# espiriki/Garbage_Classification_RCA

Hardware: AMD Instinct MI355X
Metric: train samples/sec (image+text pairs), MM-RCA ViT-B16+DistilBERT (higher is better)
Workload: dtype bf16

## Files before the change

garbage_classification_rca_amd/csrc/attention_cls.hip:

```cpp
#include "common.h"

#define CLS_MAX_S 1024
#define CLS_MAX_DH 128

template <typename T>
__device__ __forceinline__ float dot_lds(const T* __restrict__ row, const float* __restrict__ vec, int dh) {
  float a = 0.f;
  for (int d = 0; d < dh; d += 4) {
    Vec4<T> v = Vec4<T>::load(row + d);
    a += v.v[0] * vec[d] + v.v[1] * vec[d + 1] + v.v[2] * vec[d + 2] + v.v[3] * vec[d + 3];
  }
  return a;
}

__device__ __forceinline__ float block_reduce(float x, float* red, bool is_max) {
  const int wave = threadIdx.x >> 6, lane = threadIdx.x & 63;
  x = is_max ? wave_max(x) : wave_sum(x);
  __syncthreads();
  if (lane == 0) red[wave] = x;
  __syncthreads();
  return is_max ? fmaxf(fmaxf(red[0], red[1]), fmaxf(red[2], red[3])) : (red[0] + red[1] + red[2] + red[3]);
}

template <typename T>
__global__ void __launch_bounds__(256)
mha_cls_fwd_k(const T* __restrict__ qkv, const int32_t* __restrict__ key_mask, T* __restrict__ out, float* __restrict__ lse,
              int B, int H, int Smax, int dh, float scale, float drop_p, uint64_t drop_seed, const int32_t* __restrict__ cu) {
  __shared__ float qv[CLS_MAX_DH], p[CLS_MAX_S], red[4], part[4][CLS_MAX_DH];
  const float drop_sc = drop_p > 0.f ? 1.f / (1.f - drop_p) : 1.f;
  const int b = blockIdx.x / H, h = blockIdx.x % H, tid = threadIdx.x;
  const int row0 = cu ? cu[b] : b * Smax, S = cu ? cu[b + 1] - cu[b] : Smax;
  if (S <= 0) return;
  const int64_t ld = 3LL * H * dh;
  const T* Q = qkv + (int64_t)row0 * ld + h * dh;
  const T* Kp = Q + H * dh;
  const T* Vp = Kp + H * dh;
  for (int d = tid; d < dh; d += 256) qv[d] = to_f(Q[d]);
  __syncthreads();
  float m = -INFINITY;
  for (int j = tid; j < S; j += 256) {
    float s = -INFINITY;
    if (!key_mask || key_mask[row0 + j] != 0) s = dot_lds(Kp + (int64_t)j * ld, qv, dh) * scale;
    p[j] = s;
    m = fmaxf(m, s);
  }
  m = block_reduce(m, red, true);
  float l = 0.f;
  for (int j = tid; j < S; j += 256) {
    const float e = m > -INFINITY ? __expf(p[j] - m) : 0.f;
    l += e;
    p[j] = (drop_p > 0.f && mmrca_uniform(drop_seed, ((uint64_t)blockIdx.x * Smax + 0) * Smax + j) < drop_p) ? 0.f : e * drop_sc;
  }
  l = block_reduce(l, red, false);
  const float inv = l > 0.f ? 1.f / l : 0.f;
  const int ncg = dh / 4, slices = 256 / ncg;
  const int cg = tid % ncg, sl = tid / ncg;
  float o[4] = {0.f, 0.f, 0.f, 0.f};
  if (sl < slices) {
    for (int j = sl; j < S; j += slices) {
      const float pj = p[j];
      Vec4<T> v = Vec4<T>::load(Vp + (int64_t)j * ld + cg * 4);
#pragma unroll
      for (int r = 0; r < 4; ++r) o[r] += pj * v.v[r];
    }
  }
  for (int off = ncg; off < 64; off <<= 1) {
#pragma unroll
    for (int r = 0; r < 4; ++r) o[r] += __shfl_xor(o[r], off, 64);
  }
  const int wave = tid >> 6, lane = tid & 63;
  if (lane < ncg) {
#pragma unroll
    for (int r = 0; r < 4; ++r) part[wave][lane * 4 + r] = o[r];
  }
  __syncthreads();
  for (int d = tid; d < dh; d += 256)
    out[(int64_t)b * (H * dh) + h * dh + d] = from_f<T>((part[0][d] + part[1][d] + part[2][d] + part[3][d]) * inv);
  if (tid == 0) lse[blockIdx.x] = l > 0.f ? m + __logf(l) : INFINITY;
}

template <typename T>
__global__ void __launch_bounds__(256)
mha_cls_bwd_k(const T* __restrict__ qkv, const int32_t* __restrict__ key_mask, const T* __restrict__ out,
              const T* __restrict__ dout, const float* __restrict__ lse, T* __restrict__ dqkv,
              int B, int H, int Smax, int dh, float scale, float drop_p, uint64_t drop_seed, const int32_t* __restrict__ cu) {
  __shared__ float qv[CLS_MAX_DH], dov[CLS_MAX_DH], pk[CLS_MAX_S], ds[CLS_MAX_S], red[4], part[4][CLS_MAX_DH];
  const float drop_sc = drop_p > 0.f ? 1.f / (1.f - drop_p) : 1.f;
  const int b = blockIdx.x / H, h = blockIdx.x % H, tid = threadIdx.x;
  const int row0 = cu ? cu[b] : b * Smax, S = cu ? cu[b + 1] - cu[b] : Smax;
  if (S <= 0) return;
  const int64_t ld = 3LL * H * dh;
  const T* Q = qkv + (int64_t)row0 * ld + h * dh;
  const T* Kp = Q + H * dh;
  const T* Vp = Kp + H * dh;
  T* dQ = dqkv + (int64_t)row0 * ld + h * dh;
  T* dK = dQ + H * dh;
  T* dV = dK + H * dh;
  float dsum = 0.f;
  for (int d = tid; d < dh; d += 256) {
    qv[d] = to_f(Q[d]);
    const float g = to_f(dout[(int64_t)b * (H * dh) + h * dh + d]);
    dov[d] = g;
    dsum += g * to_f(out[(int64_t)b * (H * dh) + h * dh + d]);
  }
  dsum = block_reduce(dsum, red, false);
  const float Lse = lse[blockIdx.x];
  for (int j = tid; j < S; j += 256) {
    float pkj = 0.f, dsj = 0.f;
    if (!key_mask || key_mask[row0 + j] != 0) {
      const float s = dot_lds(Kp + (int64_t)j * ld, qv, dh) * scale;
      const float pj = __expf(s - Lse);
      const float dp = dot_lds(Vp + (int64_t)j * ld, dov, dh);
      const float keep = drop_p > 0.f ? (mmrca_uniform(drop_seed, ((uint64_t)blockIdx.x * Smax + 0) * Smax + j) >= drop_p ? drop_sc : 0.f) : 1.f;
      dsj = pj * (dp * keep - dsum) * scale;
      pkj = pj * keep;
    }
    pk[j] = pkj; ds[j] = dsj;
  }
  __syncthreads();
  const int ncg = dh / 4, slices = 256 / ncg;
  const int cg = tid % ncg, sl = tid / ncg;
  float qa[4] = {0.f, 0.f, 0.f, 0.f};
  if (sl < slices) {
    float dor[4], qr[4];
#pragma unroll
    for (int r = 0; r < 4; ++r) { dor[r] = dov[cg * 4 + r]; qr[r] = qv[cg * 4 + r]; }
    for (int j = sl; j < S; j += slices) {
      const float pkj = pk[j], dsj = ds[j];
      Vec4<T> k = Vec4<T>::load(Kp + (int64_t)j * ld + cg * 4), ov, ok, oz;
#pragma unroll
      for (int r = 0; r < 4; ++r) { ov.v[r] = pkj * dor[r]; ok.v[r] = dsj * qr[r]; oz.v[r] = 0.f; qa[r] += dsj * k.v[r]; }
      ov.store(dV + (int64_t)j * ld + cg * 4);
      ok.store(dK + (int64_t)j * ld + cg * 4);
      if (j > 0) oz.store(dQ + (int64_t)j * ld + cg * 4);
    }
  }
  for (int off = ncg; off < 64; off <<= 1) {
#pragma unroll
    for (int r = 0; r < 4; ++r) qa[r] += __shfl_xor(qa[r], off, 64);
  }
  const int wave = tid >> 6, lane = tid & 63;
  if (lane < ncg) {
#pragma unroll
    for (int r = 0; r < 4; ++r) part[wave][lane * 4 + r] = qa[r];
  }
  __syncthreads();
  for (int d = tid; d < dh; d += 256) dQ[d] = from_f<T>(part[0][d] + part[1][d] + part[2][d] + part[3][d]);
}

static bool cls_shape_ok(int S, int dh) {
  return S <= CLS_MAX_S && dh <= CLS_MAX_DH && (dh == 16 || dh == 32 || dh == 64 || dh == 128);
}

extern "C" int mmrca_mha_cls_fwd(const void* qkv, const int32_t* key_mask, void* out, float* lse, int B, int H, int S, int dh,
                                 float scale, float drop_p, uint64_t drop_seed, const int32_t* cu_seqlens, int dtype, void* stream) {
  MMRCA_REQUIRE(qkv && out && lse, "mha_cls_fwd: null pointer");
  MMRCA_REQUIRE(drop_p >= 0.f && drop_p < 1.f, "mha_cls_fwd: dropout p must be in [0,1)");
  MMRCA_REQUIRE(B > 0 && H > 0 && S > 0 && cls_shape_ok(S, dh), "mha_cls_fwd: B=%d H=%d S=%d dh=%d unsupported", B, H, S, dh);
  MMRCA_DISPATCH_DTYPE(dtype, "mha_cls_fwd",
    hipLaunchKernelGGL(mha_cls_fwd_k<T>, dim3(B * H), dim3(256), 0, (hipStream_t)stream, (const T*)qkv, key_mask, (T*)out, lse,
                       B, H, S, dh, scale, drop_p, drop_seed, cu_seqlens);)
  MMRCA_CHECK_LAUNCH("mha_cls_fwd");
  return 0;
}

extern "C" int mmrca_mha_cls_bwd(const void* qkv, const int32_t* key_mask, const void* out, const void* dout, const float* lse,
                                 void* dqkv, int B, int H, int S, int dh, float scale, float drop_p, uint64_t drop_seed,
                                 const int32_t* cu_seqlens, int dtype, void* stream) {
  MMRCA_REQUIRE(qkv && out && dout && lse && dqkv, "mha_cls_bwd: null pointer");
  MMRCA_REQUIRE(drop_p >= 0.f && drop_p < 1.f, "mha_cls_bwd: dropout p must be in [0,1)");
  MMRCA_REQUIRE(B > 0 && H > 0 && S > 0 && cls_shape_ok(S, dh), "mha_cls_bwd: B=%d H=%d S=%d dh=%d unsupported", B, H, S, dh);
  MMRCA_DISPATCH_DTYPE(dtype, "mha_cls_bwd",
    hipLaunchKernelGGL(mha_cls_bwd_k<T>, dim3(B * H), dim3(256), 0, (hipStream_t)stream, (const T*)qkv, key_mask, (const T*)out,
                       (const T*)dout, lse, (T*)dqkv, B, H, S, dh, scale, drop_p, drop_seed, cu_seqlens);)
  MMRCA_CHECK_LAUNCH("mha_cls_bwd");
  return 0;
}

MMRCA_SEED_EPOCH_EXPORT(attention_cls)
```

garbage_classification_rca_amd/csrc/gemm.hip:

```cpp
#include "common.h"
#include "lds_asm.h"

typedef __attribute__((ext_vector_type(4))) float f32x4;

template <typename T>
__global__ void __launch_bounds__(256)
gemm_ref_k(const T* __restrict__ A, const T* __restrict__ B, void* __restrict__ Cv, const T* __restrict__ bias,
           const T* __restrict__ addend, T* __restrict__ preact, int64_t M, int64_t N, int64_t K,
           int64_t sam, int64_t sak, int64_t sbn, int64_t sbk, int64_t ldc, int act, int accum) {
  __shared__ float As[16][65], Bs[16][65];
  const int tx = threadIdx.x & 15, ty = threadIdx.x >> 4;
  const int64_t m0 = (int64_t)blockIdx.y * 64, n0 = (int64_t)blockIdx.x * 64;
  float acc[4][4], mid[4][4];
#pragma unroll
  for (int i = 0; i < 4; ++i)
#pragma unroll
    for (int j = 0; j < 4; ++j) acc[i][j] = mid[i][j] = 0.f;
  int blk = 0;
  for (int64_t k0 = 0; k0 < K; k0 += 16) {
#pragma unroll
    for (int i = 0; i < 4; ++i) {
      const int idx = threadIdx.x + i * 256;
      int mm, kk;
      if (sak == 1) { mm = idx >> 4; kk = idx & 15; } else { kk = idx >> 6; mm = idx & 63; }
// ... 857 lines not shown
      if (seg == 2) Bp = B_lo;
    }
    if (!ATOMIC_F32 && !X3 && t == nt - 1 && ((kend - kbeg) & (GBK - 1)) != 0) {
      stage_tile<A_KROW, 1>(Ap, lda, m_blk, M, kbeg + (int64_t)t * GBK, smem, wave, lane, kend);
      stage_tile<B_KROW, 2>(Bp, ldb, n_blk, N, kbeg + (int64_t)t * GBK, smem + TILE_BYTES, wave, lane, kend);
    } else {
      stage_tile<A_KROW>(Ap, lda, m_blk, M, kbeg + (int64_t)t * GBK, smem, wave, lane);
      stage_tile<B_KROW>(Bp, ldb, n_blk, N, kbeg + (int64_t)t * GBK, smem + TILE_BYTES, wave, lane);
    }
    asm volatile("s_waitcnt vmcnt(0)" ::: "memory");
    __syncthreads();
#pragma unroll
    for (int ks = 0; ks < 2; ++ks) {
      bf16x8 af[4], bfr[4];
#pragma unroll
      for (int i = 0; i < 4; ++i) af[i] = load_frag<A_KROW>(smem, wr * 64 + i * 16, ks, lane);
#pragma unroll
      for (int j = 0; j < 4; ++j) bfr[j] = load_frag<B_KROW>(smem + TILE_BYTES, wc * 64 + j * 16, ks, lane);
#pragma unroll
      for (int i = 0; i < 4; ++i)
#pragma unroll
        for (int j = 0; j < 4; ++j) {
          if (ATOMIC_F32) acc[i][j] = __builtin_amdgcn_mfma_f32_16x16x32_bf16(af[i], bfr[j], acc[i][j], 0, 0, 0);
          else            acc[i][j] = __builtin_amdgcn_mfma_f32_16x16x32_bf16(bfr[j], af[i], acc[i][j], 0, 0, 0);
        }
    }
    __syncthreads();
  }
  const int g = lane >> 4, l16 = lane & 15;
  if (ATOMIC_F32) {
    float* C = (float*)Cv;
#pragma unroll
    for (int i = 0; i < 4; ++i)
#pragma unroll
      for (int j = 0; j < 4; ++j) {
        const int64_t n = n_blk + wc * 64 + j * 16 + l16;
#pragma unroll
        for (int r = 0; r < 4; ++r) {
          const int64_t m = m_blk + wr * 64 + i * 16 + 4 * g + r;
          if (m < M && n < N) atomicAdd(C + m * ldc + n, acc[i][j][r]);
        }
      }
  } else if constexpr (X3) {
    const float* biasf = reinterpret_cast<const float*>(bias);
    const float* addf = reinterpret_cast<const float*>(addend);
    float* pref = reinterpret_cast<float*>(preact);
    constexpr int EP_STRIDE = 128 * 4 + 16;
    const int half = lane >> 5, l32 = lane & 31;
    const int64_t ncol = n_blk + l32 * 4;
    f32x4 bv = (f32x4){0.f, 0.f, 0.f, 0.f};
    if (biasf) bv = *reinterpret_cast<const f32x4*>(biasf + ncol);
    const float* side = act == MMRCA_ACT_MUL ? pref : addf;
    float cs[4] = {0.f, 0.f, 0.f, 0.f};
#pragma unroll
    for (int i = 0; i < 4; ++i) {
      f32x4 sd[4];
      if (side) {
#pragma unroll
        for (int rr = 0; rr < 4; ++rr) {
          const int lrow = wave * 8 + rr * 2 + half;
          int64_t m = m_blk + (lrow >> 4) * 64 + i * 16 + (lrow & 15);
          if (m > M - 1) m = M - 1;
          sd[rr] = *reinterpret_cast<const f32x4*>(side + m * ldc + ncol);
        }
      }
#pragma unroll
      for (int j = 0; j < 4; ++j)
        *reinterpret_cast<f32x4*>(smem + (wr * 16 + l16) * EP_STRIDE + (wc * 64 + j * 16 + 4 * g) * 4) = acc[i][j];
      __syncthreads();
#pragma unroll
      for (int rr = 0; rr < 4; ++rr) {
        const int lrow = wave * 8 + rr * 2 + half;
        const int64_t m = m_blk + (lrow >> 4) * 64 + i * 16 + (lrow & 15);
        if (m < M && ncol < N) {
          const f32x4 c = *reinterpret_cast<const f32x4*>(smem + lrow * EP_STRIDE + l32 * 16);
          float v[4] = {c[0] + bv[0], c[1] + bv[1], c[2] + bv[2], c[3] + bv[3]};
          if (act == MMRCA_ACT_MUL) {
#pragma unroll
            for (int r = 0; r < 4; ++r) v[r] *= sd[rr][r];
          } else if (act == MMRCA_ACT_GELU_SAVE_GRAD) {
            float dg[4];
            gelu_and_grad_fast4(v, dg);
            if (pre16) {
              bf16x4 o16;
#pragma unroll
              for (int r = 0; r < 4; ++r) o16[r] = (bf16_t)dg[r];
              *reinterpret_cast<bf16x4*>(preact + m * ldc + ncol) = o16;
            } else {
              *reinterpret_cast<f32x4*>(pref + m * ldc + ncol) = (f32x4){dg[0], dg[1], dg[2], dg[3]};
            }
          } else if (act == MMRCA_ACT_GELU_BWD) {
            const f32x4 h4 = *reinterpret_cast<const f32x4*>(pref + m * ldc + ncol);
#pragma unroll
            for (int r = 0; r < 4; ++r) v[r] *= gelu_grad_f(h4[r]);
          } else if (pref) {
            *reinterpret_cast<f32x4*>(pref + m * ldc + ncol) = (f32x4){v[0], v[1], v[2], v[3]};
          }
          if (act == MMRCA_ACT_GELU) gelu_fast4(v);
          if (addf) {
            if (act == MMRCA_ACT_MUL) {
              const f32x4 a4 = *reinterpret_cast<const f32x4*>(addf + m * ldc + ncol);
#pragma unroll
              for (int r = 0; r < 4; ++r) v[r] += a4[r];
            } else {
#pragma unroll
              for (int r = 0; r < 4; ++r) v[r] += sd[rr][r];
            }
          }
          if (C_lo) {
            bf16x4 hi, lo;
#pragma unroll
            for (int r = 0; r < 4; ++r) { hi[r] = (bf16_t)v[r]; lo[r] = (bf16_t)(v[r] - (float)hi[r]); cs[r] += (float)hi[r] + (float)lo[r]; }
            *reinterpret_cast<bf16x4*>(reinterpret_cast<bf16_t*>(Cv) + m * ldc + ncol) = hi;
            *reinterpret_cast<bf16x4*>(C_lo + m * ldc + ncol) = lo;
          } else {
#pragma unroll
            for (int r = 0; r < 4; ++r) cs[r] += v[r];
            *reinterpret_cast<f32x4*>(reinterpret_cast<float*>(Cv) + m * ldc + ncol) = (f32x4){v[0], v[1], v[2], v[3]};
          }
        }
      }
      __syncthreads();
    }
    if (colsum) {
      float* red = reinterpret_cast<float*>(smem);
#pragma unroll
      for (int r = 0; r < 4; ++r) red[(wave * 2 + half) * 128 + l32 * 4 + r] = cs[r];
      __syncthreads();
      if (threadIdx.x < 128) {
        float t = 0.f;
#pragma unroll
        for (int q = 0; q < 8; ++q) t += red[q * 128 + threadIdx.x];
        if (n_blk + threadIdx.x < N) atomicAdd(colsum + n_blk + threadIdx.x, t);
      }
    }
  } else {
    bf16_t* C = (bf16_t*)Cv;
    constexpr int EP_STRIDE = 128 * 4 + 16;
    const int half = lane >> 5, l32 = lane & 31;
    const int64_t ncol = n_blk + l32 * 4;
    float bv[4] = {0.f, 0.f, 0.f, 0.f};
    if (bias) {
      bf16x4 b4 = *reinterpret_cast<const bf16x4*>(bias + (ncol < N ? ncol : N - 4));
#pragma unroll
      for (int r = 0; r < 4; ++r) bv[r] = (float)b4[r];
    }
    bf16x4 add4[4][4];
    const bf16_t* side = act == MMRCA_ACT_MUL ? preact : addend;
    if (side) {
#pragma unroll
      for (int i = 0; i < 4; ++i)
#pragma unroll
        for (int rr = 0; rr < 4; ++rr) {
          const int lrow = wave * 8 + rr * 2 + half;
          int64_t m = m_blk + (lrow >> 4) * 64 + i * 16 + (lrow & 15);
          if (m > M - 1) m = M - 1;
          add4[i][rr] = *reinterpret_cast<const bf16x4*>(side + m * ldc + ncol);
        }
    }
    float cs[4] = {0.f, 0.f, 0.f, 0.f};
    [[maybe_unused]] float st2[4] = {0.f, 0.f, 0.f, 0.f}, stsh[4] = {0.f, 0.f, 0.f, 0.f};
    if constexpr (BNS) {
      if (bst.shift && ncol < N) {
#pragma unroll
        for (int r = 0; r < 4; ++r) stsh[r] = bst.shift[ncol + r];
      }
    }
#pragma unroll
    for (int i = 0; i < 4; ++i) {
#pragma unroll
      for (int j = 0; j < 4; ++j)
        *reinterpret_cast<f32x4*>(smem + (wr * 16 + l16) * EP_STRIDE + (wc * 64 + j * 16 + 4 * g) * 4) = acc[i][j];
      __syncthreads();
#pragma unroll
      for (int rr = 0; rr < 4; ++rr) {
        const int lrow = wave * 8 + rr * 2 + half;
        const int64_t m = m_blk + (lrow >> 4) * 64 + i * 16 + (lrow & 15);
        if (m < M && ncol < N) {
          const f32x4 c = *reinterpret_cast<const f32x4*>(smem + lrow * EP_STRIDE + l32 * 16);
          float v[4] = {c[0] + bv[0], c[1] + bv[1], c[2] + bv[2], c[3] + bv[3]};
          if (act == MMRCA_ACT_MUL) {
#pragma unroll
            for (int r = 0; r < 4; ++r) v[r] *= (float)add4[i][rr][r];
          } else if (act == MMRCA_ACT_GELU_SAVE_GRAD) {
            bf16x4 o;
            float dg[4];
            gelu_and_grad_fast4(v, dg);
#pragma unroll
            for (int r = 0; r < 4; ++r) o[r] = (bf16_t)dg[r];
            *reinterpret_cast<bf16x4*>(preact + m * ldc + ncol) = o;
          } else if (act == MMRCA_ACT_GELU_BWD) {
            bf16x4 h4 = *reinterpret_cast<const bf16x4*>(preact + m * ldc + ncol);
#pragma unroll
            for (int r = 0; r < 4; ++r) v[r] *= gelu_grad_f((float)h4[r]);
          } else if (preact) {
            bf16x4 o;
#pragma unroll
            for (int r = 0; r < 4; ++r) o[r] = (bf16_t)v[r];
            *reinterpret_cast<bf16x4*>(preact + m * ldc + ncol) = o;
          }
          if (act == MMRCA_ACT_GELU) {
            gelu_fast4(v);
          }
          if (addend) {
            if (act == MMRCA_ACT_MUL) {
              bf16x4 a4 = *reinterpret_cast<const bf16x4*>(addend + m * ldc + ncol);
#pragma unroll
              for (int r = 0; r < 4; ++r) v[r] += (float)a4[r];
            } else {
#pragma unroll
              for (int r = 0; r < 4; ++r) v[r] += (float)add4[i][rr][r];
            }
          }
          bf16x4 o;
#pragma unroll
          for (int r = 0; r < 4; ++r) {
            o[r] = (bf16_t)v[r];
            if constexpr (BNS) { const float d = (float)o[r] - stsh[r]; cs[r] += d; st2[r] = fmaf(d, d, st2[r]); }
            else cs[r] += (float)o[r];
          }
          *reinterpret_cast<bf16x4*>(C + m * ldc + ncol) = o;
        }
      }
      __syncthreads();
    }
    if constexpr (BNS) {
      float* red = reinterpret_cast<float*>(smem);
#pragma unroll
      for (int r = 0; r < 4; ++r) { red[(wave * 2 + half) * 128 + l32 * 4 + r] = cs[r]; red[1024 + (wave * 2 + half) * 128 + l32 * 4 + r] = st2[r]; }
      __syncthreads();
      const int col = threadIdx.x & 127, which = threadIdx.x >> 7;
      float t = 0.f;
#pragma unroll
      for (int q = 0; q < 8; ++q) t += red[which * 1024 + q * 128 + col];
      if (n_blk + col < N) (which ? bst.s2 : bst.s1)[(int64_t)tm * N + n_blk + col] = t;
    } else if (colsum) {
      float* red = reinterpret_cast<float*>(smem);
#pragma unroll
      for (int r = 0; r < 4; ++r) red[(wave * 2 + half) * 128 + l32 * 4 + r] = cs[r];
      __syncthreads();
      if (threadIdx.x < 128) {
        float t = 0.f;
#pragma unroll
        for (int q = 0; q < 8; ++q) t += red[q * 128 + threadIdx.x];
        if (n_blk + threadIdx.x < N) atomicAdd(colsum + n_blk + threadIdx.x, t);
      }
    }
  }
}

template <bool AK, bool BK2, bool AT, int WPE, bool X3 = false, bool BNS = false, bool F4 = false>
static void launch_mfma1s(const void* A, const void* B, void* C, const void* bias, const void* addend, void* preact,
                          int64_t M, int64_t N, int64_t K, int64_t lda, int64_t ldb, int64_t ldc, int act, int tiles_m,
                          int tiles_n, int ksplits, int64_t ksplit_len, float* colsum, hipStream_t st,
                          const void* A_lo = nullptr, const void* B_lo = nullptr, void* C_lo = nullptr, int nseg = 3,
                          BnStat bst = BnStat{nullptr, nullptr, nullptr}, int pre16 = 0) {
  hipLaunchKernelGGL((gemm_mfma_k1s<AK, BK2, AT, WPE, X3, BNS, F4>), dim3(tiles_m * tiles_n, ksplits), dim3(256), 2 * TILE_BYTES, st,
                     (const bf16_t*)A, (const bf16_t*)B, C, (const bf16_t*)bias, (const bf16_t*)addend, (bf16_t*)preact,
                     M, N, K, lda, ldb, ldc, act, tiles_m, tiles_n, ksplit_len, colsum, (const bf16_t*)A_lo, (const bf16_t*)B_lo,
                     (bf16_t*)C_lo, nseg, bst, pre16);
}

static void wgrad_ksplit(int64_t K, int64_t tiles, int64_t target, int& ksplits, int64_t& ksplit_len) {
  const int64_t ksteps = K / GBK;
  int64_t want = target / tiles;
  if (want < 1) want = 1;
  if (want > ksteps / 4) want = ksteps / 4 > 0 ? ksteps / 4 : 1;
  const int64_t steps_per = (ksteps + want - 1) / want;
  ksplit_len = steps_per * GBK;
  ksplits = (int)((ksteps + steps_per - 1) / steps_per);
}

int mmrca_gemm_k1s_x3(const void* A_hi, const void* A_lo, const void* B_hi, const void* B_lo, void* C, void* C_lo, const void* bias,
                      const void* addend, void* preact, float* colsum, int64_t M, int64_t N, int64_t K, int64_t lda, int64_t ldb,
                      int64_t ldc, int a_layout, int b_layout, int act, int accum, hipStream_t st, int pre16) {
  const int tiles_m = (int)((M + GBM - 1) / GBM), tiles_n = (int)(N / GBN);
  int ksplits = 1;
  int64_t ksplit_len = K;
  if (accum) wgrad_ksplit(K, (int64_t)tiles_m * tiles_n, 1024, ksplits, ksplit_len);
  const bool ak = a_layout == MMRCA_KROW, bk = b_layout == MMRCA_KROW, at = accum != 0;
  if (A_lo && B_lo && !at && K % 32 == 0) {
    with_bools([&](auto ak_, auto bk_) {
      launch_mfma1s<ak_, bk_, false, 4, true, false, true>(A_hi, B_hi, C, bias, addend, preact, M, N, K, lda, ldb, ldc, act, tiles_m, tiles_n, 1, K,
                                                           colsum, st, A_lo, B_lo, C_lo, 3, BnStat{nullptr, nullptr, nullptr}, pre16);
    }, ak, bk);
    MMRCA_CHECK_LAUNCH("gemm_x3(k1s,fused)");
    return 0;
  }
  with_bools([&](auto ak_, auto bk_, auto at_) {
    launch_mfma1s<ak_, bk_, at_, 4, true>(A_hi, B_hi, C, bias, addend, preact, M, N, K, lda, ldb, ldc, act, tiles_m, tiles_n, ksplits, ksplit_len,
                                          colsum, st, A_lo, B_lo, C_lo, A_lo ? (B_lo ? 3 : 2) : 1, BnStat{nullptr, nullptr, nullptr}, pre16);
  }, ak, bk, at);
  MMRCA_CHECK_LAUNCH("gemm_x3(k1s)");
  return 0;
}

static bool aligned16(const void* p) { return (((uintptr_t)p) & 15) == 0; }

bool mmrca_gemm256_ok(int64_t M, int64_t N, int64_t K, int a_layout, int act, bool has_addend, bool has_preact, bool has_colsum, bool has_bias);
int mmrca_gemm256(const void* A, const void* B, void* C, const void* bias, const void* addend, void* preact, int64_t M,
                  int64_t N, int64_t K, int64_t lda, int64_t ldb, int64_t ldc, int a_layout, int b_layout, int act,
                  float* colsum, hipStream_t st);

int mmrca_gemm256_streamk_split(int64_t M, int64_t N, int64_t ksteps, void* stream, bool x3);
int64_t mmrca_gemm256_round_split(int64_t M, int64_t N);
extern int g_mmrca_dbg;

template <bool AK, bool BK2, bool AT, bool DB>
static void launch_mfma(const void* A, const void* B, void* C, const void* bias, const void* addend, void* preact,
                        int64_t M, int64_t N, int64_t K, int64_t lda, int64_t ldb, int64_t ldc, int act, int tiles_m,
                        int tiles_n, int ksplits, int64_t ksplit_len, float* dbias, hipStream_t st) {
  MMRCA_MAX_LDS(LDS128_BYTES, gemm_mfma_k<AK, BK2, AT, DB>);
  hipLaunchKernelGGL((gemm_mfma_k<AK, BK2, AT, DB>), dim3(tiles_m * tiles_n, ksplits), dim3(256), LDS128_BYTES, st,
                     (const bf16_t*)A, (const bf16_t*)B, C, (const bf16_t*)bias, (const bf16_t*)addend, (bf16_t*)preact,
                     M, N, K, lda, ldb, ldc, act, tiles_m, tiles_n, ksplit_len, dbias);
}

static int gemm_dispatch(const void* A, const void* B, void* C, const void* bias, const void* addend, void* preact,
                         int64_t M, int64_t N, int64_t K, int64_t lda, int64_t ldb, int64_t ldc,
                         int a_layout, int b_layout, int act, int out_f32_accum, int dtype, int impl, void* stream,
                         float* colsum_fused, bool* fused_done, bool rows_readable = false) {
  MMRCA_REQUIRE(A && B && C, "gemm: null operand");
  MMRCA_REQUIRE(M > 0 && N > 0 && K > 0, "gemm: bad shape M=%lld N=%lld K=%lld", (long long)M, (long long)N, (long long)K);
  MMRCA_REQUIRE((a_layout == MMRCA_ROWK || a_layout == MMRCA_KROW) && (b_layout == MMRCA_ROWK || b_layout == MMRCA_KROW), "gemm: bad layout");
  MMRCA_REQUIRE(act >= MMRCA_ACT_NONE && act <= MMRCA_ACT_MUL, "gemm: bad activation");
  MMRCA_REQUIRE(act < MMRCA_ACT_GELU_BWD || preact, "gemm: this activation needs the `preact` buffer");
  MMRCA_REQUIRE(lda >= (a_layout == MMRCA_ROWK ? K : M) && ldb >= (b_layout == MMRCA_ROWK ? K : N) && ldc >= N, "gemm: leading dimension too small");
  MMRCA_REQUIRE(!(out_f32_accum && (addend || preact || act != MMRCA_ACT_NONE)), "gemm: accumulate mode takes no epilogue");
  MMRCA_REQUIRE(!(out_f32_accum && bias && a_layout != MMRCA_KROW), "gemm: the fused bias gradient needs A in KROW layout");
  hipStream_t st = (hipStream_t)stream;

  bool ok_mfma = (dtype == MMRCA_BF16) && (N % GBN == 0) && (K % GBK == 0) && (lda % 8 == 0) && (ldb % 8 == 0) &&
                 (ldc % 4 == 0) && aligned16(A) && aligned16(B) && aligned16(C) && (!bias || aligned16(bias)) &&
                 (!addend || aligned16(addend)) && (!preact || aligned16(preact)) &&
                 (a_layout == MMRCA_ROWK || M % GBM == 0);
  const bool strict_mfma = ok_mfma;
  const bool k_ok = K % 32 == 0 || (!out_f32_accum && K % 8 == 0 && K >= 32);
  if (!ok_mfma && dtype == MMRCA_BF16 && N % 8 == 0 && N >= 8 && k_ok && (a_layout == MMRCA_ROWK || (M % 8 == 0 && M >= 8)) &&
      lda % 8 == 0 && ldb % 8 == 0 && ldc % 4 == 0 && aligned16(A) && aligned16(B) && aligned16(C) && (!bias || (aligned16(bias) && !out_f32_accum)) &&
      !addend && !preact && act == MMRCA_ACT_NONE && !colsum_fused && (out_f32_accum ? K % 64 == 0 : true) && M >= (out_f32_accum ? 16 : 64) &&
      (impl == MMRCA_GEMM_AUTO || impl == MMRCA_GEMM_MFMA_BK32 || impl == MMRCA_GEMM_MFMA_1STAGE))
    ok_mfma = true;
  const bool ragged = ok_mfma && !strict_mfma;
  const bool ok256 = strict_mfma && !out_f32_accum && mmrca_gemm256_ok(M, N, K, a_layout, act, addend != nullptr, preact != nullptr, colsum_fused != nullptr, bias != nullptr) &&
                     M * lda * 2 < (1ll << 32) && (b_layout == MMRCA_KROW ? K * ldb : N * ldb) * 2 < (1ll << 32) && M * ldc * 2 < (1ll << 32);
  if (impl == MMRCA_GEMM_MFMA256 && !ok256)
    return mmrca_fail(-3, "gemm: shape M=%lld N=%lld K=%lld does not qualify for the 256x256 MFMA kernel", (long long)M, (long long)N, (long long)K);
  if (impl == MMRCA_GEMM_MFMA256 && M % 256 != 0 && !rows_readable)
    return mmrca_fail(-4, "gemm: impl=MFMA256 with M=%lld (not a multiple of 256) reads rows up to %lld of A and of the side operand: "
                      "call mmrca_gemm_rows and state the readable row counts", (long long)M, (long long)((M + 255) / 256 * 256));
  const bool side256 = addend != nullptr || act == MMRCA_ACT_MUL;
  const bool auto256 = impl == MMRCA_GEMM_AUTO && ok256 && M % 256 == 0 && K >= 768 && (M / 256) * (N / 256) >= 256 && !side256;
  if (ok256 && (impl == MMRCA_GEMM_MFMA256 || auto256)) {
    const int64_t M1 = auto256 && !colsum_fused && mmrca_gemm256_streamk_split(M, N, K / 64, stream, false) < 2 ? mmrca_gemm256_round_split(M, N) : 0;
    if (M1 > 0) {
      if (int rc = mmrca_gemm256(A, B, C, bias, addend, preact, M1, N, K, lda, ldb, ldc, a_layout, b_layout, act, nullptr, st)) return rc;
      const char* A2 = (const char*)A + M1 * lda * 2;
      char* C2 = (char*)C + M1 * ldc * 2;
      const char* add2 = addend ? (const char*)addend + M1 * ldc * 2 : nullptr;
      char* pre2 = preact ? (char*)preact + M1 * ldc * 2 : nullptr;
      return gemm_dispatch(A2, B, C2, bias, add2, pre2, M - M1, N, K, lda, ldb, ldc, a_layout, b_layout, act, 0, dtype, MMRCA_GEMM_MFMA,
                           stream, nullptr, nullptr);
    }
    if (colsum_fused && fused_done) *fused_done = true;
    return mmrca_gemm256(A, B, C, bias, addend, preact, M, N, K, lda, ldb, ldc, a_layout, b_layout, act, colsum_fused, st);
  }
  if (impl == MMRCA_GEMM_MFMA_PERSIST || impl == MMRCA_GEMM_MFMA_TALL || impl == MMRCA_GEMM_MFMA_256W || impl == MMRCA_GEMM_MFMA_256X4)
    return mmrca_fail(-3, "gemm: impl %d was an experimental kernel of round 1 (measured slower, DESIGN.md K2) and has been removed", impl);
  if ((impl == MMRCA_GEMM_MFMA || impl == MMRCA_GEMM_MFMA_BK32 || impl == MMRCA_GEMM_MFMA_1STAGE) && !ok_mfma)
    return mmrca_fail(-3, "gemm: shape M=%lld N=%lld K=%lld dtype=%d does not qualify for the MFMA kernel", (long long)M, (long long)N, (long long)K, dtype);
  const bool use_mfma = ok_mfma && impl != MMRCA_GEMM_REF;

  if (use_mfma) {
    const int tiles_m = (int)((M + GBM - 1) / GBM), tiles_n = (int)((N + GBN - 1) / GBN);
    int ksplits = 1;
    int64_t ksplit_len = K;
    if (out_f32_accum) {
      const int64_t tiles = (int64_t)tiles_m * tiles_n;
      wgrad_ksplit(K, tiles, (g_mmrca_dbg >> 8) > 0 ? (g_mmrca_dbg >> 8) : (tiles >= 64 ? 1024 : 512), ksplits, ksplit_len);
    }
    const bool ak = a_layout == MMRCA_KROW, bk = b_layout == MMRCA_KROW, at = out_f32_accum != 0;
    const bool edge64 = impl == MMRCA_GEMM_MFMA_1STAGE && !out_f32_accum && K % 64 != 0 && K % 8 == 0 && K >= 64;
    const bool need32 = K % 64 != 0 && !edge64;
    const bool auto1s = impl == MMRCA_GEMM_AUTO && !at && !need32 &&
                        !((int64_t)tiles_m * tiles_n < 512 && K >= 768 && !colsum_fused && !ragged);
    const bool auto32 = (impl == MMRCA_GEMM_AUTO && at && (int64_t)tiles_m * tiles_n >= 64) || need32;
    if ((impl == MMRCA_GEMM_MFMA_BK32 || auto32) && !(at && bias)) {
      with_bools([&](auto ak_, auto bk_, auto at_) {
        launch_mfma32<ak_, bk_, at_>(A, B, C, bias, addend, preact, M, N, K, lda, ldb, ldc, act, tiles_m, tiles_n, ksplits, ksplit_len, st);
      }, ak, bk, at);
      MMRCA_CHECK_LAUNCH("gemm(mfma,bk32)");
      return 0;
    }
    if ((impl == MMRCA_GEMM_MFMA_1STAGE || auto1s) && !(at && bias)) {
      float* cs1 = at ? nullptr : colsum_fused;
      if (cs1 && fused_done) *fused_done = true;
      with_bools([&](auto ak_, auto bk_, auto at_) {
        launch_mfma1s<ak_, bk_, at_, 4>(A, B, C, bias, addend, preact, M, N, K, lda, ldb, ldc, act, tiles_m, tiles_n, ksplits, ksplit_len, cs1, st);
      }, ak, bk, at);
      MMRCA_CHECK_LAUNCH("gemm(mfma,1stage)");
      return 0;
    }
    if (at && bias && (impl == MMRCA_GEMM_MFMA_BK32 || auto32)) {
      with_bools([&](auto bk_) {
        launch_mfma32<true, bk_, true, true>(A, B, C, nullptr, addend, preact, M, N, K, lda, ldb, ldc, act, tiles_m, tiles_n, ksplits, ksplit_len, st, (float*)bias);
      }, bk);
      MMRCA_CHECK_LAUNCH("gemm(mfma,bk32,wgrad+dbias)");
      return 0;
    }
    if (at && bias) {
      with_bools([&](auto bk_) {
        launch_mfma<true, bk_, true, true>(A, B, C, nullptr, addend, preact, M, N, K, lda, ldb, ldc, act, tiles_m, tiles_n, ksplits, ksplit_len, (float*)bias, st);
      }, bk);
      MMRCA_CHECK_LAUNCH("gemm(mfma,wgrad+dbias)");
      return 0;
    }
    with_bools([&](auto ak_, auto bk_, auto at_) {
      launch_mfma<ak_, bk_, at_, false>(A, B, C, bias, addend, preact, M, N, K, lda, ldb, ldc, act, tiles_m, tiles_n, ksplits, ksplit_len, nullptr, st);
    }, ak, bk, at);
    MMRCA_CHECK_LAUNCH("gemm(mfma)");
    return 0;
  }

  if (out_f32_accum && bias) {
    if (int rc = mmrca_colsum_accum(A, (float*)bias, K, M, lda, dtype, stream)) return rc;
    bias = nullptr;
  }
  const int64_t sam = a_layout == MMRCA_ROWK ? lda : 1, sak = a_layout == MMRCA_ROWK ? 1 : lda;
  const int64_t sbn = b_layout == MMRCA_ROWK ? ldb : 1, sbk = b_layout == MMRCA_ROWK ? 1 : ldb;
  if (impl != MMRCA_GEMM_REF) {
    const int64_t tm = (M + 127) / 128, tn = (N + 63) / 64;
    MMRCA_REQUIRE(tm * tn < (1ll << 31), "gemm(gen): too many tiles");
    int64_t splits = 1, ksplit_len = K;
    if (out_f32_accum && tm * tn < 128 && K >= 512) {
      splits = (512 + tm * tn - 1) / (tm * tn);
      if (splits > K / 128) splits = K / 128;
      ksplit_len = ((K + splits - 1) / splits + 15) / 16 * 16;
      splits = (K + ksplit_len - 1) / ksplit_len;
    }
#define LGEN(AK_, BK_)                                                                                                            \
    MMRCA_DISPATCH_DTYPE(dtype, "gemm",                                                                                             \
      hipLaunchKernelGGL((gemm_gen_k<T, AK_, BK_>), dim3((unsigned)(tm * tn), (unsigned)splits), dim3(256), 0, st, (const T*)A,     \
                         (const T*)B, C, (const T*)bias, (const T*)addend, (T*)preact, M, N, K, sam, sak, sbn, sbk, ldc, act,     \
                         out_f32_accum, (int)tn, ksplit_len);)
    if (sak == 1 && sbk == 1) { LGEN(true, true) }
    else if (sak == 1) { LGEN(true, false) }
    else if (sbk == 1) { LGEN(false, true) }
    else { LGEN(false, false) }
#undef LGEN
    MMRCA_CHECK_LAUNCH("gemm(gen)");
    return 0;
  }
  dim3 grid((unsigned)((N + 63) / 64), (unsigned)((M + 63) / 64));
  MMRCA_REQUIRE(grid.y <= 65535, "gemm(ref): M too large for the reference kernel grid");
  MMRCA_DISPATCH_DTYPE(dtype, "gemm",
    hipLaunchKernelGGL(gemm_ref_k<T>, grid, dim3(256), 0, st, (const T*)A, (const T*)B, C, (const T*)bias, (const T*)addend,
                       (T*)preact, M, N, K, sam, sak, sbn, sbk, ldc, act, out_f32_accum);)
  MMRCA_CHECK_LAUNCH("gemm(ref)");
  return 0;
}

extern "C" int mmrca_gemm(const void* A, const void* B, void* C, const void* bias, const void* addend, void* preact,
                          int64_t M, int64_t N, int64_t K, int64_t lda, int64_t ldb, int64_t ldc,
                          int a_layout, int b_layout, int act, int out_f32_accum, int dtype, int impl, void* stream) {
  return gemm_dispatch(A, B, C, bias, addend, preact, M, N, K, lda, ldb, ldc, a_layout, b_layout, act, out_f32_accum, dtype,
                       impl, stream, nullptr, nullptr);
}

extern "C" int mmrca_gemm_colsum(const void* A, const void* B, void* C, const void* bias, const void* addend, void* preact,
                                 float* colsum, int64_t M, int64_t N, int64_t K, int64_t lda, int64_t ldb, int64_t ldc,
                                 int a_layout, int b_layout, int act, int dtype, int impl, void* stream) {
  MMRCA_REQUIRE(colsum, "gemm_colsum: null colsum");
  bool done = false;
  if (int rc = gemm_dispatch(A, B, C, bias, addend, preact, M, N, K, lda, ldb, ldc, a_layout, b_layout, act, 0, dtype, impl,
                             stream, colsum, &done))
    return rc;
  if (!done) return mmrca_colsum_accum(C, colsum, M, N, ldc, dtype, stream);
  return 0;
}

extern "C" int64_t mmrca_gemm_bnstats_slots(int64_t M) { return M > 0 ? (M + GBM - 1) / GBM : 0; }
extern "C" int mmrca_gemm_bnstats(const void* A, const void* B, void* C, int64_t M, int64_t N, int64_t K, int64_t lda, int64_t ldb, int64_t ldc,
                                  int dtype, const float* shift, float* s1, float* s2, void* stream) {
  MMRCA_REQUIRE(A && B && C && s1 && s2 && M > 0 && N > 0 && K > 0, "gemm_bnstats: bad arguments");
  MMRCA_REQUIRE(lda >= K && ldb >= K && ldc >= N, "gemm_bnstats: leading dimension too small");
  if (!(dtype == MMRCA_BF16 && N % 8 == 0 && N >= 8 && K % 32 == 0 && M >= 64 && lda % 8 == 0 && ldb % 8 == 0 && ldc % 4 == 0 &&
        aligned16(A) && aligned16(B) && aligned16(C) && (!shift || aligned16(shift))))
    return mmrca_fail(-3, "gemm_bnstats: shape M=%lld N=%lld K=%lld / dtype %d is not taken by the 128x128 bf16 kernels", (long long)M,
                      (long long)N, (long long)K, dtype);
  const int tiles_m = (int)((M + GBM - 1) / GBM), tiles_n = (int)((N + GBN - 1) / GBN);
  hipStream_t st = (hipStream_t)stream;
  const BnStat bst{shift, s1, s2};
  if (K % 64 == 0)
    launch_mfma1s<false, false, false, 4, false, true>(A, B, C, nullptr, nullptr, nullptr, M, N, K, lda, ldb, ldc, MMRCA_ACT_NONE, tiles_m, tiles_n, 1, K,
                                          nullptr, st, nullptr, nullptr, nullptr, 3, bst);
  else
    launch_mfma32<false, false, false, false, true>(A, B, C, nullptr, nullptr, nullptr, M, N, K, lda, ldb, ldc, MMRCA_ACT_NONE, tiles_m, tiles_n, 1, K, st,
                                       nullptr, bst);
  MMRCA_CHECK_LAUNCH("gemm_bnstats");
  return 0;
}

extern "C" int mmrca_gemm_rows(const void* A, const void* B, void* C, const void* bias, const void* addend, void* preact,
                               float* colsum, int64_t M, int64_t N, int64_t K, int64_t lda, int64_t ldb, int64_t ldc,
                               int64_t a_rows_readable, int64_t side_rows_readable, int a_layout, int b_layout, int act, int dtype,
                               int impl, void* stream) {
  const int64_t need = (M + 255) / 256 * 256;
  const bool has_side = addend != nullptr || act == MMRCA_ACT_MUL;
  MMRCA_REQUIRE(a_rows_readable >= M && (!has_side || side_rows_readable >= M), "gemm_rows: readable rows below M");
  bool vouched = true;
  if (impl == MMRCA_GEMM_MFMA256 && a_layout == MMRCA_ROWK) {
    if (a_rows_readable < need)
      return mmrca_fail(-4, "gemm_rows: the 256x256 kernel reads %lld rows of A, only %lld are readable", (long long)need, (long long)a_rows_readable);
    if (has_side && side_rows_readable < need)
      return mmrca_fail(-4, "gemm_rows: the 256x256 kernel reads %lld rows of the side operand, only %lld are readable", (long long)need, (long long)side_rows_readable);
  }
  bool done = false;
  if (int rc = gemm_dispatch(A, B, C, bias, addend, preact, M, N, K, lda, ldb, ldc, a_layout, b_layout, act, 0, dtype, impl, stream,
                             colsum, colsum ? &done : nullptr, vouched))
    return rc;
  if (colsum && !done) return mmrca_colsum_accum(C, colsum, M, N, ldc, dtype, stream);
  return 0;
}
```

Before: 7103.

## Add skinny-M MFMA GEMM path and cooperative dot products in CLS attention

```diff
diff --git a/garbage_classification_rca_amd/csrc/attention_cls.hip b/garbage_classification_rca_amd/csrc/attention_cls.hip
--- a/garbage_classification_rca_amd/csrc/attention_cls.hip
+++ b/garbage_classification_rca_amd/csrc/attention_cls.hip
@@ -2,16 +2,6 @@
 
 #define CLS_MAX_S 1024
 #define CLS_MAX_DH 128
-
-template <typename T>
-__device__ __forceinline__ float dot_lds(const T* __restrict__ row, const float* __restrict__ vec, int dh) {
-  float a = 0.f;
-  for (int d = 0; d < dh; d += 4) {
-    Vec4<T> v = Vec4<T>::load(row + d);
-    a += v.v[0] * vec[d] + v.v[1] * vec[d + 1] + v.v[2] * vec[d + 2] + v.v[3] * vec[d + 3];
-  }
-  return a;
-}
 
 __device__ __forceinline__ float block_reduce(float x, float* red, bool is_max) {
   const int wave = threadIdx.x >> 6, lane = threadIdx.x & 63;
@@ -37,11 +27,24 @@
   const T* Vp = Kp + H * dh;
   for (int d = tid; d < dh; d += 256) qv[d] = to_f(Q[d]);
   __syncthreads();
+  const int ncg = dh / 4, slices = 256 / ncg;
+  const int cg = tid % ncg, sl = tid / ncg;
+  float qr[4];
+#pragma unroll
+  for (int r = 0; r < 4; ++r) qr[r] = qv[cg * 4 + r];
   float m = -INFINITY;
-  for (int j = tid; j < S; j += 256) {
-    float s = -INFINITY;
-    if (!key_mask || key_mask[row0 + j] != 0) s = dot_lds(Kp + (int64_t)j * ld, qv, dh) * scale;
-    p[j] = s;
+#pragma unroll 4
+  for (int j0 = 0; j0 < S; j0 += slices) {
+    const int j = j0 + sl;
+    const bool live = j < S && (!key_mask || key_mask[row0 + j] != 0);
+    float s = 0.f;
+    if (live) {
+      Vec4<T> k = Vec4<T>::load(Kp + (int64_t)j * ld + cg * 4);
+      s = (k.v[0] * qr[0] + k.v[1] * qr[1]) + (k.v[2] * qr[2] + k.v[3] * qr[3]);
+    }
+    for (int off = 1; off < ncg; off <<= 1) s += __shfl_xor(s, off, 64);
+    s = live ? s * scale : -INFINITY;
+    if (cg == 0 && j < S) p[j] = s;
     m = fmaxf(m, s);
   }
   m = block_reduce(m, red, true);
@@ -53,16 +56,13 @@
   }
   l = block_reduce(l, red, false);
   const float inv = l > 0.f ? 1.f / l : 0.f;
-  const int ncg = dh / 4, slices = 256 / ncg;
-  const int cg = tid % ncg, sl = tid / ncg;
   float o[4] = {0.f, 0.f, 0.f, 0.f};
-  if (sl < slices) {
-    for (int j = sl; j < S; j += slices) {
-      const float pj = p[j];
-      Vec4<T> v = Vec4<T>::load(Vp + (int64_t)j * ld + cg * 4);
+#pragma unroll 4
+  for (int j = sl; j < S; j += slices) {
+    const float pj = p[j];
+    Vec4<T> v = Vec4<T>::load(Vp + (int64_t)j * ld + cg * 4);
 #pragma unroll
-      for (int r = 0; r < 4; ++r) o[r] += pj * v.v[r];
-    }
+    for (int r = 0; r < 4; ++r) o[r] += pj * v.v[r];
   }
   for (int off = ncg; off < 64; off <<= 1) {
 #pragma unroll
@@ -84,7 +84,7 @@
 mha_cls_bwd_k(const T* __restrict__ qkv, const int32_t* __restrict__ key_mask, const T* __restrict__ out,
               const T* __restrict__ dout, const float* __restrict__ lse, T* __restrict__ dqkv,
               int B, int H, int Smax, int dh, float scale, float drop_p, uint64_t drop_seed, const int32_t* __restrict__ cu) {
-  __shared__ float qv[CLS_MAX_DH], dov[CLS_MAX_DH], pk[CLS_MAX_S], ds[CLS_MAX_S], red[4], part[4][CLS_MAX_DH];
+  __shared__ float qv[CLS_MAX_DH], dov[CLS_MAX_DH], red[4], part[4][CLS_MAX_DH];
   const float drop_sc = drop_p > 0.f ? 1.f / (1.f - drop_p) : 1.f;
   const int b = blockIdx.x / H, h = blockIdx.x % H, tid = threadIdx.x;
   const int row0 = cu ? cu[b] : b * Smax, S = cu ? cu[b + 1] - cu[b] : Smax;
@@ -105,29 +105,34 @@
   }
   dsum = block_reduce(dsum, red, false);
   const float Lse = lse[blockIdx.x];
-  for (int j = tid; j < S; j += 256) {
+  const int ncg = dh / 4, slices = 256 / ncg;
+  const int cg = tid % ncg, sl = tid / ncg;
+  float qa[4] = {0.f, 0.f, 0.f, 0.f}, dor[4], qr[4];
+#pragma unroll
+  for (int r = 0; r < 4; ++r) { dor[r] = dov[cg * 4 + r]; qr[r] = qv[cg * 4 + r]; }
+#pragma unroll 2
+  for (int j0 = 0; j0 < S; j0 += slices) {
+    const int j = j0 + sl;
+    const bool live = j < S && (!key_mask || key_mask[row0 + j] != 0);
+    Vec4<T> k, ov, ok, oz;
+    float s = 0.f, dp = 0.f;
+#pragma unroll
+    for (int r = 0; r < 4; ++r) k.v[r] = 0.f;
+    if (live) {
+      k = Vec4<T>::load(Kp + (int64_t)j * ld + cg * 4);
+      Vec4<T> v = Vec4<T>::load(Vp + (int64_t)j * ld + cg * 4);
+      s = (k.v[0] * qr[0] + k.v[1] * qr[1]) + (k.v[2] * qr[2] + k.v[3] * qr[3]);
+      dp = (v.v[0] * dor[0] + v.v[1] * dor[1]) + (v.v[2] * dor[2] + v.v[3] * dor[3]);
+    }
+    for (int off = 1; off < ncg; off <<= 1) { s += __shfl_xor(s, off, 64); dp += __shfl_xor(dp, off, 64); }
     float pkj = 0.f, dsj = 0.f;
-    if (!key_mask || key_mask[row0 + j] != 0) {
-      const float s = dot_lds(Kp + (int64_t)j * ld, qv, dh) * scale;
-      const float pj = __expf(s - Lse);
-      const float dp = dot_lds(Vp + (int64_t)j * ld, dov, dh);
+    if (live) {
+      const float pj = __expf(s * scale - Lse);
       const float keep = drop_p > 0.f ? (mmrca_uniform(drop_seed, ((uint64_t)blockIdx.x * Smax + 0) * Smax + j) >= drop_p ? drop_sc : 0.f) : 1.f;
       dsj = pj * (dp * keep - dsum) * scale;
       pkj = pj * keep;
     }
-    pk[j] = pkj; ds[j] = dsj;
-  }
-  __syncthreads();
-  const int ncg = dh / 4, slices = 256 / ncg;
-  const int cg = tid % ncg, sl = tid / ncg;
-  float qa[4] = {0.f, 0.f, 0.f, 0.f};
-  if (sl < slices) {
-    float dor[4], qr[4];
-#pragma unroll
-    for (int r = 0; r < 4; ++r) { dor[r] = dov[cg * 4 + r]; qr[r] = qv[cg * 4 + r]; }
-    for (int j = sl; j < S; j += slices) {
-      const float pkj = pk[j], dsj = ds[j];
-      Vec4<T> k = Vec4<T>::load(Kp + (int64_t)j * ld + cg * 4), ov, ok, oz;
+    if (j < S) {
 #pragma unroll
       for (int r = 0; r < 4; ++r) { ov.v[r] = pkj * dor[r]; ok.v[r] = dsj * qr[r]; oz.v[r] = 0.f; qa[r] += dsj * k.v[r]; }
       ov.store(dV + (int64_t)j * ld + cg * 4);
diff --git a/garbage_classification_rca_amd/csrc/gemm.hip b/garbage_classification_rca_amd/csrc/gemm.hip
--- a/garbage_classification_rca_amd/csrc/gemm.hip
+++ b/garbage_classification_rca_amd/csrc/gemm.hip
@@ -1183,6 +1183,11 @@
                   int64_t N, int64_t K, int64_t lda, int64_t ldb, int64_t ldc, int a_layout, int b_layout, int act,
                   float* colsum, hipStream_t st);
 
+bool mmrca_gemm_skinny_ok(const void* A, const void* B, const void* C, const void* bias, const void* addend, const void* preact,
+                          int64_t M, int64_t N, int64_t K, int64_t lda, int64_t ldb, int64_t ldc, int a_layout, int dtype);
+int mmrca_gemm_skinny(const void* A, const void* B, void* C, const void* bias, const void* addend, void* preact, float* colsum,
+                      int64_t M, int64_t N, int64_t K, int64_t lda, int64_t ldb, int64_t ldc, int b_layout, int act, hipStream_t st);
+
 int mmrca_gemm256_streamk_split(int64_t M, int64_t N, int64_t ksteps, void* stream, bool x3);
 int64_t mmrca_gemm256_round_split(int64_t M, int64_t N);
 extern int g_mmrca_dbg;
@@ -1210,6 +1215,12 @@
   MMRCA_REQUIRE(!(out_f32_accum && (addend || preact || act != MMRCA_ACT_NONE)), "gemm: accumulate mode takes no epilogue");
   MMRCA_REQUIRE(!(out_f32_accum && bias && a_layout != MMRCA_KROW), "gemm: the fused bias gradient needs A in KROW layout");
   hipStream_t st = (hipStream_t)stream;
+
+  if (impl == MMRCA_GEMM_AUTO && !out_f32_accum && !(g_mmrca_dbg & 4) &&
+      mmrca_gemm_skinny_ok(A, B, C, bias, addend, preact, M, N, K, lda, ldb, ldc, a_layout, dtype)) {
+    if (colsum_fused && fused_done) *fused_done = true;
+    return mmrca_gemm_skinny(A, B, C, bias, addend, preact, colsum_fused, M, N, K, lda, ldb, ldc, b_layout, act, st);
+  }
 
   bool ok_mfma = (dtype == MMRCA_BF16) && (N % GBN == 0) && (K % GBK == 0) && (lda % 8 == 0) && (ldb % 8 == 0) &&
                  (ldc % 4 == 0) && aligned16(A) && aligned16(B) && aligned16(C) && (!bias || aligned16(bias)) &&
diff --git a/garbage_classification_rca_amd/csrc/gemm_skinny.hip b/garbage_classification_rca_amd/csrc/gemm_skinny.hip
--- /dev/null
+++ b/garbage_classification_rca_amd/csrc/gemm_skinny.hip
@@ -0,0 +1,190 @@
+#include "common.h"
+
+#define SK_BM 64
+#define SK_DEPTH 4
+#define SK_TP 72
+
+typedef __attribute__((ext_vector_type(8))) __bf16 sk_b8;
+typedef __attribute__((ext_vector_type(4))) __bf16 sk_b4;
+typedef __attribute__((ext_vector_type(4))) float sk_f4;
+
+template <bool B_KROW, int NF>
+__global__ void __launch_bounds__(256)
+gemm_skinny_k(const bf16_t* __restrict__ A, const bf16_t* __restrict__ B, bf16_t* __restrict__ C, const bf16_t* __restrict__ bias,
+              const bf16_t* __restrict__ addend, bf16_t* __restrict__ preact, int M, int N, int K, int64_t lda, int64_t ldb,
+              int64_t ldc, int act, float* __restrict__ colsum) {
+  constexpr int BN = 16 * NF, RP = BN + 4;
+  __shared__ __attribute__((aligned(16))) float red[4][SK_BM][RP];
+  __shared__ __attribute__((aligned(16))) bf16_t bt[B_KROW ? 4 : 1][B_KROW ? BN : 1][SK_TP];
+  const int t = threadIdx.x, wave = t >> 6, lane = t & 63, l16 = lane & 15, g = lane >> 4;
+  const int n0 = blockIdx.x * BN, m0 = blockIdx.y * SK_BM;
+  const int nwin = K / 64;
+  const int cnt = wave < nwin ? (nwin - wave + 3) / 4 : 0;
+
+  const bf16_t* pa[4];
+#pragma unroll
+  for (int i = 0; i < 4; ++i) {
+    int row = m0 + i * 16 + l16;
+    if (row > M - 1) row = M - 1;
+    pa[i] = A + (int64_t)row * lda + 16 * g;
+  }
+  sk_b8 ra[SK_DEPTH][4][2], rb[SK_DEPTH][2 * NF];
+  auto load = [&](int s, int step) {
+    int win = wave + 4 * step;
+    if (win > nwin - 1) win = nwin - 1;
+    const int kw = win * 64;
+#pragma unroll
+    for (int i = 0; i < 4; ++i) {
+      ra[s][i][0] = *reinterpret_cast<const sk_b8*>(pa[i] + kw);
+      ra[s][i][1] = *reinterpret_cast<const sk_b8*>(pa[i] + kw + 8);
+    }
+    if constexpr (B_KROW) {
+      const bf16_t* p = B + (int64_t)(kw + lane) * ldb + n0;
+#pragma unroll
+      for (int q = 0; q < 2 * NF; ++q) rb[s][q] = *reinterpret_cast<const sk_b8*>(p + 8 * q);
+    } else {
+#pragma unroll
+      for (int j = 0; j < NF; ++j) {
+        const bf16_t* p = B + (int64_t)(n0 + j * 16 + l16) * ldb + kw + 16 * g;
+        rb[s][2 * j] = *reinterpret_cast<const sk_b8*>(p);
+        rb[s][2 * j + 1] = *reinterpret_cast<const sk_b8*>(p + 8);
+      }
+    }
+  };
+
+  sk_f4 acc[4][NF];
+#pragma unroll
+  for (int i = 0; i < 4; ++i)
+#pragma unroll
+    for (int j = 0; j < NF; ++j) acc[i][j] = (sk_f4){0.f, 0.f, 0.f, 0.f};
+
+#pragma unroll
+  for (int s = 0; s < SK_DEPTH; ++s) load(s, s);
+  for (int it = 0; it < cnt; it += SK_DEPTH) {
+#pragma unroll
+    for (int s = 0; s < SK_DEPTH; ++s) {
+      if (it + s < cnt) {
+        sk_b8 bf[NF][2];
+        if constexpr (B_KROW) {
+          __builtin_amdgcn_fence(__ATOMIC_ACQ_REL, "wavefront");
+          __builtin_amdgcn_wave_barrier();
+#pragma unroll
+          for (int q = 0; q < 2 * NF; ++q)
+#pragma unroll
+            for (int e = 0; e < 8; ++e) bt[wave][8 * q + e][lane] = rb[s][q][e];
+          __builtin_amdgcn_fence(__ATOMIC_ACQ_REL, "wavefront");
+          __builtin_amdgcn_wave_barrier();
+#pragma unroll
+          for (int j = 0; j < NF; ++j)
+#pragma unroll
+            for (int h = 0; h < 2; ++h) bf[j][h] = *reinterpret_cast<const sk_b8*>(&bt[wave][j * 16 + l16][16 * g + 8 * h]);
+        } else {
+#pragma unroll
+          for (int j = 0; j < NF; ++j) { bf[j][0] = rb[s][2 * j]; bf[j][1] = rb[s][2 * j + 1]; }
+        }
+#pragma unroll
+        for (int h = 0; h < 2; ++h)
+#pragma unroll
+          for (int i = 0; i < 4; ++i)
+#pragma unroll
+            for (int j = 0; j < NF; ++j)
+              acc[i][j] = __builtin_amdgcn_mfma_f32_16x16x32_bf16(bf[j][h], ra[s][i][h], acc[i][j], 0, 0, 0);
+        load(s, it + s + SK_DEPTH);
+      }
+    }
+  }
+
+#pragma unroll
+  for (int i = 0; i < 4; ++i)
+#pragma unroll
+    for (int j = 0; j < NF; ++j) *reinterpret_cast<sk_f4*>(&red[wave][i * 16 + l16][j * 16 + 4 * g]) = acc[i][j];
+  __syncthreads();
+  constexpr int TPR = BN / 4, RPP = 256 / TPR;
+  const int c4 = (t % TPR) * 4, r0 = t / TPR;
+  const int ncol = n0 + c4;
+  float bv[4] = {0.f, 0.f, 0.f, 0.f};
+  if (bias) {
+    const sk_b4 b4 = *reinterpret_cast<const sk_b4*>(bias + ncol);
+#pragma unroll
+    for (int r = 0; r < 4; ++r) bv[r] = (float)b4[r];
+  }
+  float cs[4] = {0.f, 0.f, 0.f, 0.f};
+#pragma unroll
+  for (int ps = 0; ps < SK_BM / RPP; ++ps) {
+    const int row = ps * RPP + r0;
+    const int64_t m = m0 + row;
+    if (m < M) {
+      const sk_f4 p0 = *reinterpret_cast<const sk_f4*>(&red[0][row][c4]), p1 = *reinterpret_cast<const sk_f4*>(&red[1][row][c4]);
+      const sk_f4 p2 = *reinterpret_cast<const sk_f4*>(&red[2][row][c4]), p3 = *reinterpret_cast<const sk_f4*>(&red[3][row][c4]);
+      float v[4];
+#pragma unroll
+      for (int r = 0; r < 4; ++r) v[r] = (((p0[r] + p1[r]) + p2[r]) + p3[r]) + bv[r];
+      if (act == MMRCA_ACT_MUL) {
+        const sk_b4 h4 = *reinterpret_cast<const sk_b4*>(preact + m * ldc + ncol);
+#pragma unroll
+        for (int r = 0; r < 4; ++r) v[r] *= (float)h4[r];
+      } else if (act == MMRCA_ACT_GELU_SAVE_GRAD) {
+        float dg[4];
+        gelu_and_grad_fast4(v, dg);
+        sk_b4 o;
+#pragma unroll
+        for (int r = 0; r < 4; ++r) o[r] = (bf16_t)dg[r];
+        *reinterpret_cast<sk_b4*>(preact + m * ldc + ncol) = o;
+      } else if (act == MMRCA_ACT_GELU_BWD) {
+        const sk_b4 h4 = *reinterpret_cast<const sk_b4*>(preact + m * ldc + ncol);
+#pragma unroll
+        for (int r = 0; r < 4; ++r) v[r] *= gelu_grad_f((float)h4[r]);
+      } else if (preact) {
+        sk_b4 o;
+#pragma unroll
+        for (int r = 0; r < 4; ++r) o[r] = (bf16_t)v[r];
+        *reinterpret_cast<sk_b4*>(preact + m * ldc + ncol) = o;
+      }
+      if (act == MMRCA_ACT_GELU) gelu_fast4(v);
+      if (addend) {
+        const sk_b4 a4 = *reinterpret_cast<const sk_b4*>(addend + m * ldc + ncol);
+#pragma unroll
+        for (int r = 0; r < 4; ++r) v[r] += (float)a4[r];
+      }
+      sk_b4 o;
+#pragma unroll
+      for (int r = 0; r < 4; ++r) { o[r] = (bf16_t)v[r]; cs[r] += (float)o[r]; }
+      *reinterpret_cast<sk_b4*>(C + m * ldc + ncol) = o;
+    }
+  }
+  if (colsum) {
+    __syncthreads();
+    float* cr = &red[0][0][0];
+#pragma unroll
+    for (int r = 0; r < 4; ++r) cr[r0 * BN + c4 + r] = cs[r];
+    __syncthreads();
+    if (t < BN) {
+      float s = 0.f;
+      for (int q = 0; q < RPP; ++q) s += cr[q * BN + t];
+      atomicAdd(colsum + n0 + t, s);
+    }
+  }
+}
+
+static bool sk_aligned16(const void* p) { return (((uintptr_t)p) & 15) == 0; }
+
+bool mmrca_gemm_skinny_ok(const void* A, const void* B, const void* C, const void* bias, const void* addend, const void* preact,
+                          int64_t M, int64_t N, int64_t K, int64_t lda, int64_t ldb, int64_t ldc, int a_layout, int dtype) {
+  return dtype == MMRCA_BF16 && a_layout == MMRCA_ROWK && M >= 1 && M <= 256 && N % 64 == 0 && K % 64 == 0 && N < (1 << 30) &&
+         K < (1 << 30) && lda % 8 == 0 && ldb % 8 == 0 && ldc % 4 == 0 && sk_aligned16(A) && sk_aligned16(B) && sk_aligned16(C) &&
+         (!bias || sk_aligned16(bias)) && (!addend || sk_aligned16(addend)) && (!preact || sk_aligned16(preact));
+}
+
+int mmrca_gemm_skinny(const void* A, const void* B, void* C, const void* bias, const void* addend, void* preact, float* colsum,
+                      int64_t M, int64_t N, int64_t K, int64_t lda, int64_t ldb, int64_t ldc, int b_layout, int act, hipStream_t st) {
+  const int tiles_m = (int)((M + SK_BM - 1) / SK_BM);
+  const bool wide = (N / 32) * tiles_m >= cu_count();
+  with_bools([&](auto bk_, auto wide_) {
+    constexpr int NF = decltype(wide_)::value ? 2 : 1;
+    hipLaunchKernelGGL((gemm_skinny_k<decltype(bk_)::value, NF>), dim3((unsigned)(N / (16 * NF)), (unsigned)tiles_m), dim3(256), 0, st,
+                       (const bf16_t*)A, (const bf16_t*)B, (bf16_t*)C, (const bf16_t*)bias, (const bf16_t*)addend, (bf16_t*)preact,
+                       (int)M, (int)N, (int)K, lda, ldb, ldc, act, colsum);
+  }, b_layout == MMRCA_KROW, wide);
+  MMRCA_CHECK_LAUNCH("gemm(skinny)");
+  return 0;
+}
```

Result: no change. 7142, median of 6 (+0.6%).
